# Niema-Lab/AmpliPy

Hardware: AMD Instinct MI355X
Metric: aligned reads/s through trim+pileup+call, 30 kb ref @ 10k x depth (higher is better)
Workload: dtype u8/int32

## Files before the change

amplipy_amd/csrc/amp_bf.hpp:

```cpp
#pragma once

#include "amp_read.hpp"

namespace amp {

struct Bf {
    int32_t a, m1, k, m2, c, kind;
    uint32_t op;
    uint32_t punt;
    AMP_HD int32_t kI() const { return kind == 1 ? k : 0; }
    AMP_HD int32_t kD() const { return kind == 2 ? k : 0; }
    AMP_HD int32_t query_len() const { return a + m1 + kI() + m2 + c; }
    AMP_HD int32_t ref_len() const { const int32_t r = m1 + m2 + kD(); return r ? r : 1; }
};
AMP_HD int32_t bf_sel(bool c, int32_t x, int32_t y) { return c ? x : y; }
AMP_HD int32_t bf_min(int32_t x, int32_t y) { return x < y ? x : y; }
AMP_HD int32_t bf_max(int32_t x, int32_t y) { return x > y ? x : y; }
AMP_HD Bf bf_pick(bool c, const Bf &x, const Bf &y) {
    return Bf{c ? x.a : y.a, c ? x.m1 : y.m1, c ? x.k : y.k, c ? x.m2 : y.m2, c ? x.c : y.c, c ? x.kind : y.kind, c ? x.op : y.op, c ? x.punt : y.punt};
}
AMP_HD Bf bf_mirror(const Bf &s) { return Bf{s.c, s.kind ? s.m2 : s.m1, s.k, s.kind ? s.m1 : s.m2, s.a, s.kind, s.op, s.punt}; }

AMP_HD Bf bf_from_words5(int n, uint32_t w0, uint32_t w1, uint32_t w2, uint32_t w3, uint32_t w4, int32_t lseq, int32_t max_ins, int32_t max_del, bool &ok) {
    const bool lead = (w0 & 15u) == OP_S;
// ... 31 lines not shown
    r = in2 ? s.a + s.m1 + s.kI() + u : r;
    r = inD ? s.a + s.m1 : r;
    r = in1 ? s.a + t : r;
    return r;
}

AMP_HD int32_t bf_ref_offset(const Bf &s, int32_t qp) {
    const bool in0 = (s.a > 0) & (qp <= s.a);
    const int32_t x = qp - s.a;
    const bool in1 = !in0 & (s.m1 > 0) & (x <= s.m1);
    const int32_t x2 = x - s.m1;
    const bool inI = !in0 & !in1 & (s.kind == 1) & (x2 <= s.k);
    const int32_t x3 = x2 - s.kI();
    const bool in2 = !in0 & !in1 & !inI & (s.kind != 0) & (s.m2 > 0) & (x3 <= s.m2);
    int32_t r = s.m1 + s.kD() + (s.kind ? s.m2 : 0);
    r = in2 ? s.m1 + s.kD() + x3 : r;
    r = inI ? s.m1 : r;
    r = in1 ? x : r;
    r = in0 ? 0 : r;
    return r;
}

template <bool QUALITY>
AMP_HD Bf bf_clip_left(const Bf &s, int32_t d, int32_t &adv) {
    const bool r1 = (s.m1 > 0) & (d < s.m1);
    const int32_t d1 = d - s.m1, A = s.a + s.m1;
    const bool stopI = !r1 & (s.kind == 1) & (d1 < s.k) & (QUALITY | (d1 > 0));
    const bool stopD = !r1 & (s.kind == 2) & (d1 == 0) & QUALITY;
    const bool stop = stopI | stopD;
    const int32_t d2 = s.kind == 1 ? bf_max(d1 - s.k, 0) : d1;
    const int32_t m = s.kind ? s.m2 : 0;
    const int32_t t = bf_min(d2, m);
    const int32_t m_left = m - t;
    const int32_t A4 = A + s.kI() + t;
    Bf o;
    o.op = s.op;
    o.punt = s.punt | ((!r1 & (s.kind != 0) & (s.m2 == 0)) ? 1u : 0u);
    o.a = r1 ? s.a + d : (stop ? A + (stopI ? d1 : 0) : A4 + (m_left == 0 ? s.c : 0));
    o.m1 = r1 ? s.m1 - d : (stop ? 0 : m_left);
    o.k = r1 ? s.k : (stop ? s.k - (stopI ? d1 : 0) : 0);
    o.m2 = (r1 | stop) ? s.m2 : 0;
    o.kind = (r1 | stop) ? s.kind : 0;
    o.c = (r1 | stop) ? s.c : (m_left == 0 ? 0 : s.c);
    adv = r1 ? d : (stop ? s.m1 : s.m1 + s.kD() + t);
    return o;
}

AMP_HD Bf bf_primer_clip(const Bf &s, int32_t del, int32_t &adv) {
    const int32_t d = s.a > 0 ? bf_max(del - s.a, 0) : del;
    int32_t adv_c;
    const Bf c = bf_clip_left<false>(s, bf_max(d, 0), adv_c);
    const bool neg = del < 0, zero = del == 0;
    Bf o;
    o.op = s.op;
    o.punt = (neg | zero) ? s.punt : c.punt;
    o.a = neg ? s.query_len() : (zero ? s.a : c.a);
    o.m1 = neg ? 0 : (zero ? s.m1 : c.m1);
    o.k = neg ? 0 : (zero ? s.k : c.k);
    o.m2 = neg ? 0 : (zero ? s.m2 : c.m2);
    o.c = neg ? 0 : (zero ? s.c : c.c);
    o.kind = neg ? 0 : (zero ? s.kind : c.kind);
    adv = neg ? s.kD() : (zero ? 0 : adv_c);
    return o;
}
AMP_HD Bf bf_canon(const Bf &s) {
    const bool all = (s.kind == 0) & (s.m1 == 0);
    Bf o = s;
    o.a = all ? s.a + s.c : s.a;
    o.c = all ? 0 : s.c;
    return o;
}

AMP_HD Bf bf_trim_primers(const Bf &s0, int32_t &pos, uint32_t &flags, uint32_t flag, bool isize_flag, int32_t lseq,
                          int32_t left_max_end, int32_t right_min_start) {
    const bool is_paired = flag & 1u, is_reverse = (flag & 0x10u) != 0;
    const bool do1 = !(is_paired & isize_flag & is_reverse) & (left_max_end >= 0);
    int32_t adv1;
    const Bf c1 = bf_primer_clip(s0, bf_pos_on_query(s0, left_max_end + 1 - pos), adv1);
    Bf s = bf_pick(do1, c1, s0);
    pos += do1 ? adv1 : 0;
    flags |= do1 ? AMP_TRIM_PRIMER_START : 0u;
    const bool do2 = !(is_paired & isize_flag & !is_reverse) & (right_min_start >= 0) & !s.punt;
    const int32_t del2 = lseq - bf_pos_on_query(s, right_min_start - pos);
    int32_t adv2;
    const Bf c2 = bf_canon(bf_mirror(bf_primer_clip(bf_mirror(s), del2, adv2)));
    flags |= do2 ? AMP_TRIM_PRIMER_END : 0u;
    return bf_pick(do2, c2, s);
}

AMP_HD void bf_quality_window(const Bf &s, int32_t lseq, int32_t &lo, int32_t &qlen) {
    const bool single = (s.m1 == 0) & (s.kind == 0);
    const int32_t qe = single ? lseq : lseq - s.c;
    lo = bf_min(s.a, lseq);
    qlen = bf_max(qe, lo) - lo;
}

AMP_HD Bf bf_trim_quality(const Bf &s, int32_t pos, uint32_t &flags, bool is_reverse, int32_t i, int32_t qlen) {
    int32_t adv;
    const int32_t del_r = i;
    const bool do_r = is_reverse & (bf_ref_offset(s, del_r + s.a - 1) > 0);
    const Bf cr = bf_clip_left<true>(s, del_r, adv);
    const Bf cr0 = bf_pick(del_r == 0, s, cr);
    const int32_t del_f = qlen - i;
    const bool do_f = !is_reverse & (del_f != 0);
    const Bf cf = bf_canon(bf_mirror(bf_clip_left<true>(bf_mirror(s), del_f, adv)));
    flags |= (do_r | do_f) ? AMP_TRIM_QUALITY : 0u;
    (void)pos;
    return bf_pick(do_r, cr0, bf_pick(do_f, cf, s));
}

}
```

amplipy_amd/csrc/amp_fast.hpp:

```cpp
#pragma once

#include "amp_tile.hpp"
#include "amp_bf.hpp"

namespace amp {

#ifndef AMP_F_LDSPAD
#define AMP_F_LDSPAD 0
#endif
#ifndef AMP_F4_LEAN
#define AMP_F4_LEAN 1
#endif
#ifndef AMP_F4_BF
#define AMP_F4_BF 1
#endif
__device__ __forceinline__ Bf bf_of(const Cig2 &s) { return Bf{s.a, s.m1, s.k, s.m2, s.c, s.kind, s.op, s.punt ? 1u : 0u}; }
__device__ __forceinline__ Cig2 cig2_of(const Bf &b) { return Cig2{b.op, b.a, b.m1, b.k, b.m2, b.c, b.kind, b.punt != 0u}; }
constexpr int F_NP = 10;
constexpr int F_MAXLEN = 152;
constexpr int F_PW = 256;
#ifndef AMP_F_REPS
#define AMP_F_REPS 8
#endif
constexpr int F_REP = AMP_F_REPS;
// ... 170 lines not shown
    const uint32_t se0 = __builtin_amdgcn_perm(0x00000010u, 0x00080018u, (sq.x >> 4) & 0x07070707u);
    const uint32_t so0 = __builtin_amdgcn_perm(0x00000010u, 0x00080018u, sq.x & 0x07070707u);
    const uint32_t se1 = __builtin_amdgcn_perm(0x00000010u, 0x00080018u, (sq.y >> 4) & 0x07070707u);
    const uint32_t so1 = __builtin_amdgcn_perm(0x00000010u, 0x00080018u, sq.y & 0x07070707u);
    const uint32_t f0 = nibble_to_bytes(m, 0), f1 = nibble_to_bytes(m, 1), f2 = nibble_to_bytes(m, 2), f3 = nibble_to_bytes(m, 3);
    const uint32_t wb = wrep + (inwin ? (uint32_t)d0 * 4u : 0u);
#define F_SH(d, sh, js, v, jv) "v_lshlrev_b32_sdwa " d ", " sh ", " v " dst_sel:DWORD dst_unused:UNUSED_PAD src0_sel:BYTE_" #js " src1_sel:BYTE_" #jv "\n\t"
#define F_AD(t, off) "ds_add_u32 %2, " t " offset:" #off "\n\t"
    {
        uint32_t t0, t1;
        asm volatile(F_SH("%0", "%3", 0, "%7", 0) F_SH("%1", "%4", 0, "%7", 1) F_AD("%0", 0) F_SH("%0", "%3", 1, "%7", 2) F_AD("%1", 4) F_SH("%1", "%4", 1, "%7", 3)
                     F_AD("%0", 8) F_SH("%0", "%3", 2, "%8", 0) F_AD("%1", 12) F_SH("%1", "%4", 2, "%8", 1) F_AD("%0", 16) F_SH("%0", "%3", 3, "%8", 2)
                     F_AD("%1", 20) F_SH("%1", "%4", 3, "%8", 3) F_AD("%0", 24) F_SH("%0", "%5", 0, "%9", 0) F_AD("%1", 28) F_SH("%1", "%6", 0, "%9", 1)
                     F_AD("%0", 32) F_SH("%0", "%5", 1, "%9", 2) F_AD("%1", 36) F_SH("%1", "%6", 1, "%9", 3) F_AD("%0", 40) F_SH("%0", "%5", 2, "%10", 0)
                     F_AD("%1", 44) F_SH("%1", "%6", 2, "%10", 1) F_AD("%0", 48) F_SH("%0", "%5", 3, "%10", 2) F_AD("%1", 52) F_SH("%1", "%6", 3, "%10", 3)
                     F_AD("%0", 56) "ds_add_u32 %2, %1 offset:60"
                     : "=&v"(t0), "=&v"(t1) : "v"(wb), "v"(se0), "v"(so0), "v"(se1), "v"(so1), "v"(f0), "v"(f1), "v"(f2), "v"(f3) : "memory");
    }
#undef F_SH
#undef F_AD
    return redo ? 1u : 0u;
}
__device__ __forceinline__ uint32_t count_piece5q(const uint2 &sq, uint32_t m16, int32_t d0, int32_t lim16, uint32_t wrep, uint32_t ooff) {
    const bool inwin = (d0 >= 0) & (d0 <= lim16);
    const bool redo = (m16 != 0u) & (!inwin | (nibbles_bad(sq.x, sq.y) != 0u));
    const uint32_t m = redo ? 0u : m16;
    const uint32_t se0 = __builtin_amdgcn_perm(0x00000010u, 0x00080018u, (sq.x >> 4) & 0x07070707u);
    const uint32_t so0 = __builtin_amdgcn_perm(0x00000010u, 0x00080018u, sq.x & 0x07070707u);
    const uint32_t se1 = __builtin_amdgcn_perm(0x00000010u, 0x00080018u, (sq.y >> 4) & 0x07070707u);
    const uint32_t so1 = __builtin_amdgcn_perm(0x00000010u, 0x00080018u, sq.y & 0x07070707u);
    const uint32_t f0 = nibble_to_bytes(m, 0), f1 = nibble_to_bytes(m, 1), f2 = nibble_to_bytes(m, 2), f3 = nibble_to_bytes(m, 3);
    const uint32_t wb = wrep + (inwin ? (uint32_t)d0 * 4u + (((uint32_t)d0 & 1u) ? ooff : 0u) : 0u);
#define F_SH(d, sh, js, v, jv) "v_lshlrev_b32_sdwa " d ", " sh ", " v " dst_sel:DWORD dst_unused:UNUSED_PAD src0_sel:BYTE_" #js " src1_sel:BYTE_" #jv "\n\t"
#define F_AQ(t, off) "ds_add_u64 %0, " t " offset:" #off "\n\t"
    asm volatile(F_SH("v252", "%1", 0, "%5", 0) F_SH("v253", "%2", 0, "%5", 1) F_AQ("v[252:253]", 0)
                 F_SH("v254", "%1", 1, "%5", 2) F_SH("v255", "%2", 1, "%5", 3) F_AQ("v[254:255]", 8)
                 F_SH("v252", "%1", 2, "%6", 0) F_SH("v253", "%2", 2, "%6", 1) F_AQ("v[252:253]", 16)
                 F_SH("v254", "%1", 3, "%6", 2) F_SH("v255", "%2", 3, "%6", 3) F_AQ("v[254:255]", 24)
                 F_SH("v252", "%3", 0, "%7", 0) F_SH("v253", "%4", 0, "%7", 1) F_AQ("v[252:253]", 32)
                 F_SH("v254", "%3", 1, "%7", 2) F_SH("v255", "%4", 1, "%7", 3) F_AQ("v[254:255]", 40)
                 F_SH("v252", "%3", 2, "%8", 0) F_SH("v253", "%4", 2, "%8", 1) F_AQ("v[252:253]", 48)
                 F_SH("v254", "%3", 3, "%8", 2) F_SH("v255", "%4", 3, "%8", 3) "ds_add_u64 %0, v[254:255] offset:56"
                 : : "v"(wb), "v"(se0), "v"(so0), "v"(se1), "v"(so1), "v"(f0), "v"(f1), "v"(f2), "v"(f3) : "memory", "v252", "v253", "v254", "v255");
#undef F_SH
#undef F_AQ
    return redo ? 1u : 0u;
}
__device__ __forceinline__ uint32_t range_bits16(int32_t klo, int32_t khi) {
    klo = klo < 0 ? 0 : (klo > 16 ? 16 : klo); khi = khi > 16 ? 16 : (khi < 0 ? 0 : khi);
    return ((1u << khi) - 1u) & ~((1u << klo) - 1u);
}

#if defined(AMP_DEV) && (!defined(AMP_ABL) || defined(AMP_ABL_STAMPS))
#define F_DBG_PARAM , uint32_t *f_dbg
#define F_GLOB ++f_glob
#define F_EPIW(k) do { __builtin_amdgcn_s_waitcnt(0x4F74); f_epw[0] = wall_clock64(); __builtin_amdgcn_s_waitcnt(0x0F7A); f_epw[1] = wall_clock64(); __builtin_amdgcn_s_waitcnt(0); f_ep[k] = wall_clock64(); } while (0)
#define F_EPI(k) do { __builtin_amdgcn_s_waitcnt(0); f_ep[k] = wall_clock64(); } while (0)
#define F_DBG_ARG(x) , (x)
#define F_STAMP_DECL unsigned long long f_t[8] = {0, 0, 0, 0, 0, 0, 0, 0}, f_prev = __builtin_amdgcn_s_memtime(); const unsigned long long f_k0 = f_prev, f_w0 = wall_clock64(); unsigned long long f_ep[3] = {0, 0, 0}, f_epw[2] = {0, 0}; uint32_t f_glob = 0
#define F_STAMP(k) do { __builtin_amdgcn_sched_barrier(0); __builtin_amdgcn_s_waitcnt(0xC07F); unsigned long long f_n = __builtin_amdgcn_s_memtime(); f_t[k] += f_n - f_prev; f_prev = f_n; __builtin_amdgcn_sched_barrier(0); } while (0)
#define F_STAMP_VM(k) do { __builtin_amdgcn_sched_barrier(0); __builtin_amdgcn_s_waitcnt(0x0070); unsigned long long f_n = __builtin_amdgcn_s_memtime(); f_t[k] += f_n - f_prev; f_prev = f_n; __builtin_amdgcn_sched_barrier(0); } while (0)
#define F_STAMP_OUT do { f_t[0] = __builtin_amdgcn_s_memtime() - f_k0; const unsigned long long f_w1 = wall_clock64(); f_t[7] = f_w1 - f_w0; if (lane == 0) { unsigned long long *const ctr = late_ctr(); for (int k = 0; k < 8; ++k) atomicAdd(&ctr[CTR_PHASE0 + k], f_t[k]); \
    atomicMax(&ctr[CTR_STAMP0], f_t[7]); atomicMax(&ctr[CTR_STAMP0 + 1], ~f_t[7]); atomicMax(&ctr[CTR_STAMP0 + 2], ~f_w0); atomicMax(&ctr[CTR_STAMP0 + 3], f_w1); \
    if (f_dbg && wave == 0) { uint32_t *f_o = f_dbg + blockIdx.x * 8; f_o[0] = (uint32_t)f_t[7]; f_o[1] = (uint32_t)f_w0; for (int k = 1; k < 7; ++k) f_o[1 + k] = (uint32_t)(f_t[k] >> 4); } \
    if (f_dbg) { uint32_t *f_o = f_dbg + F_DBG_WAVE0 + (blockIdx.x * F_WAVES + wave) * F_DBG_WAVEWORDS; f_o[0] = (uint32_t)((f_t[1] + f_t[2] + f_t[3] + f_t[4] + f_t[5] + f_t[6]) >> 4); f_o[1] = (uint32_t)(f_epw[0] - f_w0); f_o[2] = (uint32_t)(f_epw[1] - f_epw[0]); f_o[3] = (uint32_t)(f_ep[0] - f_epw[1]); f_o[4] = (uint32_t)(f_ep[1] - f_ep[0]); f_o[5] = (uint32_t)(f_ep[2] - f_ep[1]); } } } while (0)
#else
#define F_DBG_PARAM
#define F_DBG_ARG(x)
#define F_GLOB
// ... 4 lines not shown
#define F_STAMP_VM(k)
#define F_STAMP_OUT
#endif

#define F_ARGS \
    const int32_t *a_pos, int32_t a_min_quality, const uint16_t *a_flag, int32_t a_window, const int32_t *a_tlen, int32_t a_do_trim, \
    const uint32_t *a_lseq, int32_t a_do_count, const uint32_t *a_cig_off32, int32_t a_ref_len, const uint32_t *a_cig, int32_t a_max_primer_len, \
    const uint32_t *a_seq_off8, int32_t reads_per_block, const uint8_t *a_seq, int32_t a_epoch, const uint8_t *a_qual, int32_t pad1, \
    const int32_t *a_min_start, int32_t pad2, const int32_t *a_max_end, int32_t pad3, \
    int32_t *a_new_pos, int32_t pad4, uint32_t *a_new_ncig, int32_t pad5, uint32_t *a_new_cig, int32_t pad6, int32_t *a_o_ref_len, int32_t pad7, \
    uint8_t *a_trim_flags, int32_t pad8, uint8_t *a_status, int32_t pad9, \
    uint32_t *counts, int32_t pad10, amp_ins_event *a_ev, int32_t pad11, unsigned long long *a_ctr, int32_t pad12, uint32_t *a_ins_at, int32_t pad13, \
    uint32_t *glist, int32_t pad14, uint32_t *gcnt, int32_t pad15, \
    int64_t a_n_reads, int32_t pad17, uint64_t read_base, int32_t pad18, long long a_ev_cap
#define F_ARGS_PASS(P, rd, out, eb, rpb) \
    (rd).pos, (P).min_quality, (rd).flag, (P).window, (rd).tlen, (P).do_trim, (rd).lseq, (P).do_count, (rd).cig_off32, (P).ref_len, (rd).cig, \
    (P).max_primer_len, (rd).seq_off8, (rpb), (rd).seq, (int32_t)(P).epoch, (rd).qual, 0, (P).min_start, 0, (P).max_end, 0, (out).new_pos, 0, (out).new_ncig, 0, \
    (out).new_cig, 0, (out).ref_len, 0, (out).trim_flags, 0, (out).status, 0, counts, 0, (eb).ev, 0, (eb).ctr, 0, (eb).ins_at, 0, glist, 0, gcnt, 0, \
    (rd).n_reads, 0, read_base, 0, (eb).cap

enum : uint32_t { KA_MIN_START = 144, KA_MAX_END = 160, KA_NEW_POS = 176, KA_NEW_NCIG = 192, KA_NEW_CIG = 208, KA_O_REF_LEN = 224, KA_TRIM_FLAGS = 240,
                  KA_STATUS = 256, KA_COUNTS = 272, KA_EV = 288, KA_CTR = 304, KA_INS_AT = 320, KA_GLIST = 336, KA_GCNT = 352, KA_N_READS = 368,
                  KA_READ_BASE = 384, KA_EV_CAP = 400 };
template <typename T>
__device__ __forceinline__ T karg_late(uint32_t off) {
    static_assert(sizeof(T) == 8, "the late-loaded arguments are pointers and 64-bit values");
    asm volatile("" : "+s"(off));
    const unsigned long long v = *(const __attribute__((address_space(4))) unsigned long long *)
        ((const __attribute__((address_space(4))) uint8_t *)__builtin_amdgcn_kernarg_segment_ptr() + off);
    return __builtin_bit_cast(T, v);
}
template <typename T>
__device__ __forceinline__ T *karg_late_ptr(uint32_t off) {
    return (T *)karg_late<__attribute__((address_space(1))) T *>(off);
}

#if AMP_F_ADD64
#define F_COUNT5(sq, m, d0, lim, wr) count_piece5q(sq, m, d0, lim, wr, (uint32_t)(F_REPW * 4))
#else
#define F_COUNT5(sq, m, d0, lim, wr) count_piece5(sq, m, d0, lim, wr)
#endif
template <int W>
__global__ void __launch_bounds__(F_WAVES * 64, 2)
k_fast(F_ARGS F_DBG_PARAM) {
    const KParams P{a_min_quality, a_window, a_do_trim, a_do_count, a_ref_len, a_max_primer_len, nullptr, nullptr, (uint32_t)a_epoch};
    const amp_dev_reads rd{a_n_reads, a_pos, a_flag, a_tlen, a_lseq, a_cig_off32, a_cig, a_seq_off8, a_seq, a_qual, 0, 0};
    auto late_ctr = [] { return karg_late_ptr<unsigned long long>(KA_CTR); };
    auto late_eb = [] { return EventBuf{karg_late_ptr<amp_ins_event>(KA_EV), karg_late_ptr<unsigned long long>(KA_CTR), karg_late_ptr<uint32_t>(KA_INS_AT), karg_late<long long>(KA_EV_CAP)}; };
    __shared__ uint4 s_stage[F_WAVES][(F_PAD + F_STAGE + 16) / 16];
    __shared__ __attribute__((aligned(8))) uint32_t s_pwin[F_WAVES][F_REP * F_REPW];
    __shared__ uint32_t s_bwin[F_BPL * F_BW];
    __shared__ uint32_t s_ticket, s_gcur;
#if AMP_F_LDSPAD > 0
    __shared__ uint32_t s_pad[AMP_F_LDSPAD / 4];
    if (P.ref_len == -12345) s_pad[threadIdx.x] = 1;
#endif
    const int tid = threadIdx.x, wave = tid >> 6, lane = tid & 63;
    F_STAMP_DECL;
    const int64_t n = rd.n_reads;
    const int64_t rb = (int64_t)blockIdx.x * reads_per_block;
    const int64_t re = rb + reads_per_block < n ? rb + reads_per_block : n;
    lds_u32 *const bwin = (lds_u32 *)s_bwin;
    lds_u32 *const pwin = (lds_u32 *)s_pwin[wave];
    for (int i = tid; i < F_BPL * F_BW; i += F_WAVES * 64) bwin[i] = 0;
    for (int i = lane; i < F_REP * F_REPW; i += 64) pwin[i] = 0;
    if (lane < F_PAD / 4) ((lds_u32 *)s_stage[wave])[lane] = 0x11111111u;
    if (tid == 0) { s_ticket = 0; s_gcur = 0; }
    if (tid == 0 && blockIdx.x == 0) { unsigned long long *const ctr = late_ctr(); ctr[CTR_LONG_N] = 0ull; ctr[CTR_LONG_TICKET] = 0ull; ctr[CTR_GEN_LEFT] = 0ull; }
    int32_t bw_base = rb < n ? rd.pos[rb] : 0;
    bw_base = (bw_base < 16 ? 0 : bw_base - 16) & ~15;
    __syncthreads();

    const int32_t mq = P.min_quality;
    const uint32_t mqc = (uint32_t)(mq > 256 ? 256 : mq);
    const uint32_t thr = mqc * (uint32_t)W;
    const uint32_t mqb = (uint32_t)mq * 0x01010101u;
    const uint32_t G = (uint32_t)P.ref_len;
    const uint32_t n_tb = re > rb ? (uint32_t)((re - rb + 63) / 64) : 0u;
    auto take_ticket = [&]() {
        uint32_t t = 0;
        if (lane == 0) t = __hip_atomic_fetch_add((lds_u32 *)&s_ticket, 1u, __ATOMIC_RELAXED, __HIP_MEMORY_SCOPE_WORKGROUP);
        return (uint32_t)__builtin_amdgcn_readfirstlane((int)t);
    };
    const int64_t wend = re;
    unsigned long long n_err = 0;
#ifndef AMP_F_REPSHIFT
#define AMP_F_REPSHIFT 2
#endif
    const uint32_t rep = (F_REP & (F_REP - 1)) ? ((uint32_t)lane >> AMP_F_REPSHIFT) % (uint32_t)F_REP : ((uint32_t)lane >> AMP_F_REPSHIFT) & (uint32_t)(F_REP - 1);
    const uint32_t phi_lane = ((uint32_t)lane >> 1) & 1u ? 8u : 0u;
#if AMP_F_ADD64
    lds_u8 *const wrep = (lds_u8 *)pwin + (rep & (uint32_t)(F_REP / 2 - 1)) * (uint32_t)(2 * F_REPW * 4);
    static_assert((F_REP & 1) == 0 && (F_REPW & 1) == 1, "two arrays per replica, the second one an odd number of words behind the first");
#else
    lds_u8 *const wrep = (lds_u8 *)pwin + rep * (uint32_t)(F_REPW * 4);
#endif
    lds_u8 *const stage = (lds_u8 *)s_stage[wave] + F_PAD;
    int32_t pw_base = 0;
    int pw_tiles = F_FLUSH;
    const unsigned ev_shard = blockIdx.x & (EV_SHARDS - 1);
    unsigned long long ev_base = 0;
    uint32_t ev_left = 0;

    auto fold = [&]() {
        asm volatile("s_waitcnt lgkmcnt(0)" ::: "memory");
        wave_sync();
#pragma unroll 1
        for (int idx = lane; idx < F_PW; idx += 64) {
// ... 80 lines not shown
        g.Tq = g.solo ? 0u : (uint32_t)__builtin_amdgcn_readlane((int)(g.row + 8u * nch), g.ntake - 1);
        g.fastq = g.taken && shortq;
        return g;
    };
    auto shape_of = [&](const HdrP &h, const Cg &c, bool fastq) {
        Shape r;
#if AMP_F4_BF
        bool ok;
        r.s = cig2_of(bf_from_words5((int)h.nops(), c.w[0], c.w[1], c.w[2], c.w[3], c.w[4], fastq ? (int32_t)h.lseq() : 0, F_MAXINS, F_MAXDEL, ok));
        r.ok = ok;
#else
        r.s = Cig2{0u, 0, 0, 0, 0, 0, 0, false};
        const int nops = (int)h.nops();
        r.ok = fastq && nops >= 1 && nops <= 5 && cig2_from_words5(nops, c.w, (int32_t)h.lseq(), r.s);
        if (r.ok && ((r.s.kind == 1 && r.s.k > F_MAXINS) || (r.s.kind == 2 && r.s.k > F_MAXDEL))) r.ok = false;
        if (!r.ok) r.s = Cig2{0u, 0, 0, 0, 0, 0, 0, false};
#endif
        r.refspan = r.ok ? r.s.m1 + r.s.m2 + (r.s.kind == 2 ? r.s.k : 0) : 1;
        return r;
    };
    auto load_tabs = [&](const HdrP &h, const Shape &sh, bool trim) {
        Tabs t{-1, -1};
        const bool in_ref = (uint32_t)h.pos < G && (uint32_t)(h.pos + sh.refspan - 1) < G;
        if (trim && in_ref) { t.L = karg_late_ptr<const int32_t>(KA_MAX_END)[h.pos]; t.R = karg_late_ptr<const int32_t>(KA_MIN_START)[h.pos + sh.refspan - 1]; }
        return t;
    };
    auto issue_bytes = [&](const Geo &g, uint32_t m0) {
        Bytes x;
        const uint8_t *qrun = rd.qual + (int64_t)m0 * 8;
        const uint8_t *srun = rd.seq + (int64_t)m0 * 4;
        const uint32_t lastq = g.Tq ? (g.Tq - 1u) & ~15u : 0u, lasts = g.Tq ? ((g.Tq >> 1) - 1u) & ~15u : 0u;
#pragma unroll
        for (int sl = 0; sl < F_STAGE / 1024; ++sl) {
            uint32_t off = (uint32_t)(sl * 1024 + lane * 16);
            off = off < lastq ? off : lastq;
            __builtin_amdgcn_global_load_lds((const __attribute__((address_space(1))) void *)(qrun + off),
                                             (__attribute__((address_space(3))) void *)(stage + sl * 1024), 16, 0, 0);
        }
#pragma unroll
        for (int sl = 0; sl < F_STAGE / 2048; ++sl) {
            uint32_t off = (uint32_t)(sl * 1024 + lane * 16);
            off = off < lasts ? off : lasts;
            const uint32_t *sp = (const uint32_t *)(srun + off);
            x.raws[sl] = make_uint4(sp[0], sp[1], sp[2], sp[3]);
        }
        return x;
    };
    enum : uint32_t { P_STORED = 1u << 24, P_LIST = 1u << 25, P_STATUS_ONLY = 1u << 26 };
    struct Pend { uint32_t i, slot_lo; int32_t pos, reflen; uint32_t meta, cw0, cw1, cw2, cw3, cw4; };
    Pend pend{0u, 0u, 0, 0, 0u, 0u, 0u, 0u, 0u, 0u};
    auto store_pending = [&](const Pend &r) {
#if defined(AMP_DEV) && defined(AMP_ABL)
        if (AMP_ABL & 8) return;
#endif
        const uint32_t ncig = r.meta & 0xFFu;
        if (r.meta & P_STORED) {
            const DevOut out{karg_late_ptr<int32_t>(KA_NEW_POS), karg_late_ptr<uint32_t>(KA_NEW_NCIG), karg_late_ptr<uint32_t>(KA_NEW_CIG),
                             karg_late_ptr<int32_t>(KA_O_REF_LEN), karg_late_ptr<uint8_t>(KA_TRIM_FLAGS), karg_late_ptr<uint8_t>(KA_STATUS)};
            uint32_t *home = out.new_cig + ((size_t)r.slot_lo + 3 * (size_t)r.i);
            if (ncig > 0u) home[0] = r.cw0;
            if (ncig > 1u) home[1] = r.cw1;
            if (ncig > 2u) home[2] = r.cw2;
            if (ncig > 3u) home[3] = r.cw3;
            if (ncig > 4u) home[4] = r.cw4;
            if (out.new_pos) out.new_pos[r.i] = r.pos;
            if (out.new_ncig) out.new_ncig[r.i] = ncig;
            if (out.ref_len) out.ref_len[r.i] = r.reflen;
            if (out.trim_flags) out.trim_flags[r.i] = (uint8_t)(r.meta >> 16);
            if (out.status) out.status[r.i] = (uint8_t)(r.meta >> 8);
        }
        const bool has = (r.meta & P_LIST) != 0;
        const unsigned long long m = __ballot(has);
        if (m) {
            uint32_t base = 0;
            if (lane == 0) base = __hip_atomic_fetch_add((lds_u32 *)&s_gcur, (uint32_t)__popcll(m), __ATOMIC_RELAXED, __HIP_MEMORY_SCOPE_WORKGROUP);
            base = (uint32_t)__builtin_amdgcn_readfirstlane((int)base);
            if (has) karg_late_ptr<uint32_t>(KA_GLIST)[(size_t)rb + base + __popcll(m & ((1ull << lane) - 1ull))] = r.i | ((r.meta & P_STATUS_ONLY) ? GL_STATUS_ONLY : 0u);
        }
    };

    uint32_t pw_lim = 0;
// ... 146 lines not shown
        if (do_trim_t && !(AMP_ABL & 4)) {
#else
        if (do_trim_t) {
#endif
#pragma unroll
            for (int k = 0; k < F_NP; ++k) {
                uint32_t p = (uint32_t)k + rot;
                p = p >= np ? p - np : p;
                p = (uint32_t)k < np ? p : np;
                const int32_t j0 = (int32_t)(p * 16u);
                uint2 nx = make_uint2(q16[0].x, q16[0].y);
                if (k + 1 < F_NP && (uint32_t)(k + 1) < np) nx = make_uint2(q16[k + 1].x, q16[k + 1].y);
                uint32_t fail = piece_fail_bits<W>(q16[k], nx, thr);
                int32_t blo = lo - j0, bhi = hi - W - j0;
                blo = blo < 0 ? 0 : (blo > 16 ? 16 : blo); bhi = bhi > 15 ? 15 : (bhi < -1 ? -1 : bhi);
                fail &= (0xFFFFu >> (15 - bhi)) & (0xFFFFu << blo);
                const int32_t f1 = j0 + (__builtin_ffs((int)fail) - 1), e1 = j0 + (31 - __builtin_clz(fail)) + W;
                ffmin = fail && f1 < ffmin ? f1 : ffmin;
                lemax = fail && e1 > lemax ? e1 : lemax;
            }
        }

        F_STAMP(3);
        bool general = i < re && !shaped;
        bool stored = false;
        uint32_t ncig = 0, cw[5] = {0u, 0u, 0u, 0u, 0u};
        int32_t reflen = 0;
        if (shaped) {
            if (fb == 0xFFu || s.punt) {
                general = true;
            } else {
                if (scan) {
                    int32_t iq;
                    if (!rev && ffmin != 0x7FFFFFFF) iq = ffmin - lo;
                    else if (rev && lemax >= 0) iq = lemax - lo;
                    else {
                        iq = rev ? 0 : qlen;
                        int32_t acc = 0;
                        const uint64_t t_lo = (uint64_t)tw0.x | ((uint64_t)tw0.y << 32), t_hi = (uint64_t)tw1.x | ((uint64_t)tw1.y << 32);
                        const int32_t kmax = qlen < W - 1 ? qlen : W - 1;
                        const int32_t qlo = lo - (int32_t)phi, qhi = hi - (int32_t)phi;
                        for (int32_t k = 1; k <= kmax; ++k) {
                            const uint32_t o = (uint32_t)((rev ? qlo + k - 1 : qhi - k) - tab);
                            acc += (int32_t)(((o < 8u ? t_lo : t_hi) >> ((o & 7u) * 8u)) & 0xFFu);
                            if ((int64_t)acc < (int64_t)mq * k) iq = rev ? k : qlen - k;
                        }
                    }
#if AMP_F4_BF
                    { uint32_t f2 = ts.flags; s = cig2_of(bf_trim_quality(bf_of(s), ts.pos, f2, rev, iq, qlen)); ts.flags = f2; }
#else
                    cig2_trim_quality(ts, rev, iq, qlen, s);
#endif
                }
                if (s.punt) {
                    general = true;
                } else {
                    if (!ts.err) {
                        const uint32_t part[5] = {((uint32_t)s.a << 4) | OP_S, ((uint32_t)s.m1 << 4) | s.op,
                                                  ((uint32_t)s.k << 4) | (s.kind == 1 ? OP_I : OP_D), ((uint32_t)s.m2 << 4) | s.op,
                                                  ((uint32_t)s.c << 4) | OP_S};
                        const bool has[5] = {s.a > 0, s.m1 > 0, s.kind != 0, s.kind != 0 && s.m2 > 0, s.c > 0};
#pragma unroll
                        for (int t = 0; t < 5; ++t) {
                            if (has[t]) {
#pragma unroll
                                for (int j = (t == 3 ? 1 : 0); j <= t; ++j) cw[j] = ncig == (uint32_t)j ? part[t] : cw[j];
                                ++ncig;
                            }
                        }
                        reflen = s.ref_len();
                    }
                    stored = true;
                    if (ts.err) ++n_err;
                }
            }
        }
        const bool counted = stored && !ts.err && do_count_t;
        F_STAMP(4);
        const bool two = counted && s.kind != 0;
        const int32_t qa1 = counted ? s.a + (int32_t)phi : 0, qb1 = counted ? qa1 + s.m1 : 0;
        const int32_t qa2 = two ? qb1 + (s.kind == 1 ? s.k : 0) : qb1, qb2 = two ? qa2 + s.m2 : qa2;
        const int32_t pos2 = ts.pos + s.m1 + (s.kind == 2 ? s.k : 0);
        bool bad_extra = false;
        if (two && s.kind == 2) {
            for (int32_t j = 0; j < s.k; ++j) {
                const int32_t r = ts.pos + s.m1 + j;
                const uint32_t d = (uint32_t)(r - bw_base);
                if ((uint32_t)r >= G) bad_extra = true;
                else if (d < (uint32_t)F_BW) lds_add_nt(bwin + 4 * F_BW + d, 1u);
                else atomicAdd(&karg_late_ptr<uint32_t>(KA_COUNTS)[(size_t)r * AMP_NSYM + 5], 1u);
            }
        }
        {
            uint32_t good = 0;
            if (two && s.kind == 1) {
                const uint32_t o0 = ok_bits4(iq0.x, mqb) >> 7, o1 = ok_bits4(iq0.y, mqb) >> 7, o2 = ok_bits4(iq1.x, mqb) >> 7, o3 = ok_bits4(iq1.y, mqb) >> 7;
                auto nib = [](uint32_t o) { return ((o * 0x00204081u) >> 21) & 0xFu; };
                const uint32_t m16 = nib(o0) | (nib(o1) << 4) | (nib(o2) << 8) | (nib(o3) << 12);
                good = (m16 >> (uint32_t)(s.a + s.m1 - g_ins)) & ((1u << s.k) - 1u);
// ... 28 lines not shown
                        if (firstrun) {
                            if ((long long)slot < eb.cap) eb.ev[(size_t)ev_shard * (size_t)eb.cap + slot] = inside ? amp_ins_event{ins_pos, rid, elo, ehi} : amp_ins_event{-1, 0u, 0, 0};
                            if (inside) {
                                const uint32_t d = (uint32_t)(ins_pos - bw_base);
                                if (d < (uint32_t)F_BW) lds_add_nt(bwin + 5 * F_BW + d, 1u);
                                else atomicAdd(&eb.ins_at[ins_pos], 1u);
                            }
                        } else if (inside) {
                            eb.record(ins_pos, rid, elo, ehi);
                        }
                        firstrun = false;
                    }
                }
                ev_base += total; ev_left -= total;
            }
        }
        uint32_t redo = 0;
#if AMP_F4_LEAN
        uint32_t okm[F_NP];
#pragma unroll
        for (int k = 0; k < F_NP; ++k) okm[k] = ok_bits16(q16[k], mqb);
        const uint32_t okB = ok_bits16(make_uint4(bq0.x, bq0.y, bq1.x, bq1.y), mqb);
#endif
        int32_t xbe = 0, jb = 0;
        bool has_b = false;
        if (two) {
            const int32_t jstar = (qb1 - 1) & ~15;
            has_b = jstar + 16 > qa2 && qb2 > qa2;
            xbe = qb2 < jstar + 16 ? qb2 : jstar + 16;
            jb = g_b + (int32_t)phi;
        }
        const int32_t end_pos = two ? pos2 + s.m2 : ts.pos + s.m1;
        bool todo = counted;
#if defined(AMP_DEV) && defined(AMP_ABL)
        if (AMP_ABL & 2) todo = false;
#endif
        for (bool first_pass = true;; first_pass = false) {
            const unsigned long long tm = __ballot(todo);
            if (!tm) break;
            const int lead = __builtin_ctzll(tm);
            if (!first_pass) {
                fold();
                const int32_t lead_pos = __builtin_amdgcn_readlane(pos, lead);
                pw_base = (lead_pos < 16 ? 0 : lead_pos - 16) & ~15; pw_tiles = 1;
                pw_lim = (int64_t)G - pw_base >= (int64_t)F_PW ? (uint32_t)F_PW : (uint32_t)(G > (uint32_t)pw_base ? G - (uint32_t)pw_base : 0u);
            }
            const bool fits = ts.pos - pw_base >= 16 && end_pos - pw_base + 16 <= (int32_t)pw_lim;
            const bool now = todo && (fits || lane == lead);
            const int32_t a1 = now ? qa1 : 0, b1 = now ? qb1 : 0, a2 = now ? qa2 : 0, b2 = now ? qb2 : 0;
            const int32_t dbase1 = ts.pos - pw_base - qa1, dbase2 = pos2 - pw_base - qa2;
#if AMP_F4_LEAN
            const int32_t lim16 = (int32_t)pw_lim - 16;
            if (__ballot(has_b && now)) {
                const uint32_t mB = (has_b & now) ? okB & range_bits16(qa2 - jb, xbe - jb) : 0u;
// ... 64 lines not shown
    store_pending(pend);
    pad_events();
    F_EPI(1);
    if (pw_tiles && n_tb) fold();
    F_EPI(2);
    asm volatile("s_waitcnt lgkmcnt(0)" ::: "memory");
    __syncthreads();
#if defined(AMP_DEV) && defined(AMP_ABL)
    if (AMP_ABL & 16) return;
#endif
    uint32_t *const counts_l = karg_late_ptr<uint32_t>(KA_COUNTS), *const ins_at_l = karg_late_ptr<uint32_t>(KA_INS_AT);
    for (int i = tid; i < F_BPL * F_BW; i += F_WAVES * 64) {
        const uint32_t v = bwin[i];
        if (v) {
            const int pl = i / F_BW, d = i - pl * F_BW;
            const uint32_t p = (uint32_t)(bw_base + d);
            if (p < G) {
                if (pl < F_NPL) atomicAdd(&counts_l[(size_t)p * AMP_NSYM + pl], v);
                else if (pl == 4) atomicAdd(&counts_l[(size_t)p * AMP_NSYM + 5], v);
                else atomicAdd(&ins_at_l[p], v);
            }
        }
    }
    if (n_err) atomicAdd(&late_ctr()[CTR_ERROR_READS], n_err);
    F_STAMP_OUT;
    if (tid == 0) { karg_late_ptr<uint32_t>(KA_GCNT)[blockIdx.x] = s_gcur; if (s_gcur) late_ctr()[CTR_EPOCH] = (unsigned long long)P.epoch; }
}

__global__ void __launch_bounds__(256)
k_gcompact(const uint32_t *__restrict__ glist, const uint32_t *__restrict__ gcnt, int reads_per_block, int64_t n_reads,
           uint32_t *__restrict__ dense, GenGeo *geo, uint32_t gen_grid, unsigned long long *ctr,
           const uint32_t *__restrict__ cig_off32, uint32_t *__restrict__ llist, uint32_t *__restrict__ lpos, int long_max_ops) {
    __shared__ uint32_t s_part[4], s_lw[4], s_lbase;
    const int tid = threadIdx.x;
    uint32_t acc = 0;
    for (int b = tid; b < (int)blockIdx.x; b += 256) acc += gcnt[b];
    for (int o = 32; o > 0; o >>= 1) acc += __shfl_down(acc, o);
    if ((tid & 63) == 0) s_part[tid >> 6] = acc;
    __syncthreads();
    const uint32_t off = s_part[0] + s_part[1] + s_part[2] + s_part[3];
    const uint32_t cnt = gcnt[blockIdx.x];
    const int64_t sbeg = (int64_t)blockIdx.x * reads_per_block;
    const uint32_t *src = glist + (sbeg < n_reads ? sbeg : 0);
    for (uint32_t k = tid; k < cnt; k += 256) dense[off + k] = src[k];
    if (long_max_ops) {
        const auto kind = [&](uint32_t k) -> uint32_t {
            if (k >= cnt) return 0u;
// ... 68 lines not shown
```

Before: 10.31 billion.

## Branchless trim/CIGAR packing, shared clip path, and paired kernarg pointer loads

Rewrites the breakpoint-form clip and trim helpers so the primer and quality trims run one clip instead of two and select between results. The mirror is made conditional, so forward and reverse share one code path. Turns the per-read CIGAR word emission and the quality-scan branching into straight-line predicated code, and fetches pairs of late kernel-argument pointers with a single 32-byte scalar load. The aim is less divergence, fewer instructions and fewer scalar loads per read, at the cost of subtle semantic equivalence risk in the clip logic and always running the quality trim math.

```diff
diff --git a/amplipy_amd/csrc/amp_bf.hpp b/amplipy_amd/csrc/amp_bf.hpp
--- a/amplipy_amd/csrc/amp_bf.hpp
+++ b/amplipy_amd/csrc/amp_bf.hpp
@@ -77,45 +77,34 @@
 }
 
 template <bool QUALITY>
-AMP_HD Bf bf_clip_left(const Bf &s, int32_t d, int32_t &adv) {
-    const bool r1 = (s.m1 > 0) & (d < s.m1);
-    const int32_t d1 = d - s.m1, A = s.a + s.m1;
-    const bool stopI = !r1 & (s.kind == 1) & (d1 < s.k) & (QUALITY | (d1 > 0));
-    const bool stopD = !r1 & (s.kind == 2) & (d1 == 0) & QUALITY;
-    const bool stop = stopI | stopD;
-    const int32_t d2 = s.kind == 1 ? bf_max(d1 - s.k, 0) : d1;
-    const int32_t m = s.kind ? s.m2 : 0;
-    const int32_t t = bf_min(d2, m);
-    const int32_t m_left = m - t;
-    const int32_t A4 = A + s.kI() + t;
+AMP_HD Bf bf_clip_left(const Bf &s, int32_t d, bool skip, int32_t &adv) {
+    const int32_t kI = s.kI(), kD = s.kD();
+    const int32_t e = bf_min(d, s.m1), d1 = d - e;
+    const int32_t kq = QUALITY ? (s.kind == 2 ? 1 : kI) : kI;
+    const bool keep = QUALITY ? ((d < s.m1 + kq) | skip) : (((d < s.m1 + kq) & (d != s.m1)) | skip);
+    const int32_t t = bf_min(bf_max(d1 - kI, 0), s.m2);
+    const int32_t m_left = s.m2 - t;
+    const bool gone = m_left == 0;
     Bf o;
     o.op = s.op;
-    o.punt = s.punt | ((!r1 & (s.kind != 0) & (s.m2 == 0)) ? 1u : 0u);
-    o.a = r1 ? s.a + d : (stop ? A + (stopI ? d1 : 0) : A4 + (m_left == 0 ? s.c : 0));
-    o.m1 = r1 ? s.m1 - d : (stop ? 0 : m_left);
-    o.k = r1 ? s.k : (stop ? s.k - (stopI ? d1 : 0) : 0);
-    o.m2 = (r1 | stop) ? s.m2 : 0;
-    o.kind = (r1 | stop) ? s.kind : 0;
-    o.c = (r1 | stop) ? s.c : (m_left == 0 ? 0 : s.c);
-    adv = r1 ? d : (stop ? s.m1 : s.m1 + s.kD() + t);
+    o.punt = s.punt | (((d >= s.m1) & !skip & (s.kind != 0) & (s.m2 == 0)) ? 1u : 0u);
+    o.a = keep ? s.a + d : s.a + s.m1 + kI + t + (gone ? s.c : 0);
+    o.m1 = keep ? s.m1 - e : m_left;
+    o.k = keep ? s.k - d1 : 0;
+    o.m2 = keep ? s.m2 : 0;
+    o.kind = keep ? s.kind : 0;
+    o.c = (keep | !gone) ? s.c : 0;
+    adv = keep ? e : s.m1 + kD + t;
     return o;
 }
 
 AMP_HD Bf bf_primer_clip(const Bf &s, int32_t del, int32_t &adv) {
-    const int32_t d = s.a > 0 ? bf_max(del - s.a, 0) : del;
+    const bool neg = del < 0, zero = del == 0;
+    const int32_t d = neg ? 0x3FFFFFFF : bf_max(del - s.a, 0);
     int32_t adv_c;
-    const Bf c = bf_clip_left<false>(s, bf_max(d, 0), adv_c);
-    const bool neg = del < 0, zero = del == 0;
-    Bf o;
-    o.op = s.op;
-    o.punt = (neg | zero) ? s.punt : c.punt;
-    o.a = neg ? s.query_len() : (zero ? s.a : c.a);
-    o.m1 = neg ? 0 : (zero ? s.m1 : c.m1);
-    o.k = neg ? 0 : (zero ? s.k : c.k);
-    o.m2 = neg ? 0 : (zero ? s.m2 : c.m2);
-    o.c = neg ? 0 : (zero ? s.c : c.c);
-    o.kind = neg ? 0 : (zero ? s.kind : c.kind);
-    adv = neg ? s.kD() : (zero ? 0 : adv_c);
+    Bf o = bf_clip_left<false>(s, d, zero, adv_c);
+    o.punt = neg ? s.punt : o.punt;
+    adv = neg ? s.kD() : adv_c;
     return o;
 }
 AMP_HD Bf bf_canon(const Bf &s) {
@@ -125,43 +114,41 @@
     o.c = all ? 0 : s.c;
     return o;
 }
+AMP_HD Bf bf_mirror_if(bool f, const Bf &s) {
+    const bool sw = f & (s.kind != 0);
+    return Bf{f ? s.c : s.a, sw ? s.m2 : s.m1, s.k, sw ? s.m1 : s.m2, f ? s.a : s.c, s.kind, s.op, s.punt};
+}
 
 AMP_HD Bf bf_trim_primers(const Bf &s0, int32_t &pos, uint32_t &flags, uint32_t flag, bool isize_flag, int32_t lseq,
                           int32_t left_max_end, int32_t right_min_start) {
     const bool is_paired = flag & 1u, is_reverse = (flag & 0x10u) != 0;
-    const bool do1 = !(is_paired & isize_flag & is_reverse) & (left_max_end >= 0);
+    const bool far = is_paired & isize_flag;
+    const bool do1 = !(far & is_reverse) & (left_max_end >= 0);
     int32_t adv1;
-    const Bf c1 = bf_primer_clip(s0, bf_pos_on_query(s0, left_max_end + 1 - pos), adv1);
-    Bf s = bf_pick(do1, c1, s0);
-    pos += do1 ? adv1 : 0;
+    const Bf s = bf_primer_clip(s0, do1 ? bf_pos_on_query(s0, left_max_end + 1 - pos) : 0, adv1);
+    pos += adv1;
     flags |= do1 ? AMP_TRIM_PRIMER_START : 0u;
-    const bool do2 = !(is_paired & isize_flag & !is_reverse) & (right_min_start >= 0) & !s.punt;
-    const int32_t del2 = lseq - bf_pos_on_query(s, right_min_start - pos);
+    const bool do2 = !(far & !is_reverse) & (right_min_start >= 0) & !s.punt;
+    const int32_t del2 = do2 ? lseq - bf_pos_on_query(s, right_min_start - pos) : 0;
     int32_t adv2;
-    const Bf c2 = bf_canon(bf_mirror(bf_primer_clip(bf_mirror(s), del2, adv2)));
     flags |= do2 ? AMP_TRIM_PRIMER_END : 0u;
-    return bf_pick(do2, c2, s);
+    return bf_canon(bf_mirror(bf_primer_clip(bf_mirror(s), del2, adv2)));
 }
 
 AMP_HD void bf_quality_window(const Bf &s, int32_t lseq, int32_t &lo, int32_t &qlen) {
-    const bool single = (s.m1 == 0) & (s.kind == 0);
-    const int32_t qe = single ? lseq : lseq - s.c;
     lo = bf_min(s.a, lseq);
-    qlen = bf_max(qe, lo) - lo;
+    qlen = bf_max(lseq - s.c, lo) - lo;
 }
 
 AMP_HD Bf bf_trim_quality(const Bf &s, int32_t pos, uint32_t &flags, bool is_reverse, int32_t i, int32_t qlen) {
     int32_t adv;
-    const int32_t del_r = i;
-    const bool do_r = is_reverse & (bf_ref_offset(s, del_r + s.a - 1) > 0);
-    const Bf cr = bf_clip_left<true>(s, del_r, adv);
-    const Bf cr0 = bf_pick(del_r == 0, s, cr);
-    const int32_t del_f = qlen - i;
-    const bool do_f = !is_reverse & (del_f != 0);
-    const Bf cf = bf_canon(bf_mirror(bf_clip_left<true>(bf_mirror(s), del_f, adv)));
-    flags |= (do_r | do_f) ? AMP_TRIM_QUALITY : 0u;
+    const bool fwd = !is_reverse;
+    const int32_t del = fwd ? qlen - i : i;
+    const bool doit = fwd ? del != 0 : bf_ref_offset(s, del + s.a - 1) > 0;
+    flags |= doit ? AMP_TRIM_QUALITY : 0u;
+    const int32_t d = doit ? del : 0;
     (void)pos;
-    return bf_pick(do_r, cr0, bf_pick(do_f, cf, s));
+    return bf_canon(bf_mirror_if(fwd, bf_clip_left<true>(bf_mirror_if(fwd, s), d, d == 0, adv)));
 }
 
 }
diff --git a/amplipy_amd/csrc/amp_fast.hpp b/amplipy_amd/csrc/amp_fast.hpp
--- a/amplipy_amd/csrc/amp_fast.hpp
+++ b/amplipy_amd/csrc/amp_fast.hpp
@@ -216,9 +216,9 @@
     return redo ? 1u : 0u;
 }
 __device__ __forceinline__ uint32_t count_piece5q(const uint2 &sq, uint32_t m16, int32_t d0, int32_t lim16, uint32_t wrep, uint32_t ooff) {
-    const bool inwin = (d0 >= 0) & (d0 <= lim16);
-    const bool redo = (m16 != 0u) & (!inwin | (nibbles_bad(sq.x, sq.y) != 0u));
-    const uint32_t m = redo ? 0u : m16;
+    const bool inwin = (uint32_t)d0 < (lim16 < 0 ? 0u : (uint32_t)lim16 + 1u);
+    const uint32_t defect = inwin ? nibbles_bad(sq.x, sq.y) : 1u;
+    const uint32_t m = defect ? 0u : m16;
     const uint32_t se0 = __builtin_amdgcn_perm(0x00000010u, 0x00080018u, (sq.x >> 4) & 0x07070707u);
     const uint32_t so0 = __builtin_amdgcn_perm(0x00000010u, 0x00080018u, sq.x & 0x07070707u);
     const uint32_t se1 = __builtin_amdgcn_perm(0x00000010u, 0x00080018u, (sq.y >> 4) & 0x07070707u);
@@ -238,7 +238,8 @@
                  : : "v"(wb), "v"(se0), "v"(so0), "v"(se1), "v"(so1), "v"(f0), "v"(f1), "v"(f2), "v"(f3) : "memory", "v252", "v253", "v254", "v255");
 #undef F_SH
 #undef F_AQ
-    return redo ? 1u : 0u;
+    const uint32_t left = m16 ^ m;
+    return left < 1u ? left : 1u;
 }
 __device__ __forceinline__ uint32_t range_bits16(int32_t klo, int32_t khi) {
     klo = klo < 0 ? 0 : (klo > 16 ? 16 : klo); khi = khi > 16 ? 16 : (khi < 0 ? 0 : khi);
@@ -289,6 +290,8 @@
 enum : uint32_t { KA_MIN_START = 144, KA_MAX_END = 160, KA_NEW_POS = 176, KA_NEW_NCIG = 192, KA_NEW_CIG = 208, KA_O_REF_LEN = 224, KA_TRIM_FLAGS = 240,
                   KA_STATUS = 256, KA_COUNTS = 272, KA_EV = 288, KA_CTR = 304, KA_INS_AT = 320, KA_GLIST = 336, KA_GCNT = 352, KA_N_READS = 368,
                   KA_READ_BASE = 384, KA_EV_CAP = 400 };
+static_assert(KA_MAX_END == KA_MIN_START + 16 && KA_NEW_NCIG == KA_NEW_POS + 16 && KA_O_REF_LEN == KA_NEW_CIG + 16 && KA_STATUS == KA_TRIM_FLAGS + 16 &&
+              KA_CTR == KA_EV + 16, "karg_late2 reads two neighbours");
 template <typename T>
 __device__ __forceinline__ T karg_late(uint32_t off) {
     static_assert(sizeof(T) == 8, "the late-loaded arguments are pointers and 64-bit values");
@@ -297,9 +300,21 @@
         ((const __attribute__((address_space(4))) uint8_t *)__builtin_amdgcn_kernarg_segment_ptr() + off);
     return __builtin_bit_cast(T, v);
 }
+struct KargPair { unsigned long long a, b; };
+__device__ __forceinline__ KargPair karg_late2(uint32_t off) {
+    typedef unsigned long long amp_u64x4 __attribute__((ext_vector_type(4), aligned(16)));
+    asm volatile("" : "+s"(off));
+    const amp_u64x4 v = *(const __attribute__((address_space(4))) amp_u64x4 *)
+        ((const __attribute__((address_space(4))) uint8_t *)__builtin_amdgcn_kernarg_segment_ptr() + off);
+    return KargPair{v.x, v.z};
+}
 template <typename T>
 __device__ __forceinline__ T *karg_late_ptr(uint32_t off) {
     return (T *)karg_late<__attribute__((address_space(1))) T *>(off);
+}
+template <typename T>
+__device__ __forceinline__ T *karg_ptr_of(unsigned long long v) {
+    return (T *)__builtin_bit_cast(__attribute__((address_space(1))) T *, v);
 }
 
 #if AMP_F_ADD64
@@ -313,7 +328,10 @@
     const KParams P{a_min_quality, a_window, a_do_trim, a_do_count, a_ref_len, a_max_primer_len, nullptr, nullptr, (uint32_t)a_epoch};
     const amp_dev_reads rd{a_n_reads, a_pos, a_flag, a_tlen, a_lseq, a_cig_off32, a_cig, a_seq_off8, a_seq, a_qual, 0, 0};
     auto late_ctr = [] { return karg_late_ptr<unsigned long long>(KA_CTR); };
-    auto late_eb = [] { return EventBuf{karg_late_ptr<amp_ins_event>(KA_EV), karg_late_ptr<unsigned long long>(KA_CTR), karg_late_ptr<uint32_t>(KA_INS_AT), karg_late<long long>(KA_EV_CAP)}; };
+    auto late_eb = [] {
+        const KargPair ec = karg_late2(KA_EV);
+        return EventBuf{karg_ptr_of<amp_ins_event>(ec.a), karg_ptr_of<unsigned long long>(ec.b), karg_late_ptr<uint32_t>(KA_INS_AT), karg_late<long long>(KA_EV_CAP)};
+    };
     __shared__ uint4 s_stage[F_WAVES][(F_PAD + F_STAGE + 16) / 16];
     __shared__ __attribute__((aligned(8))) uint32_t s_pwin[F_WAVES][F_REP * F_REPW];
     __shared__ uint32_t s_bwin[F_BPL * F_BW];
@@ -350,7 +368,7 @@
         return (uint32_t)__builtin_amdgcn_readfirstlane((int)t);
     };
     const int64_t wend = re;
-    unsigned long long n_err = 0;
+    uint32_t n_err = 0;
 #ifndef AMP_F_REPSHIFT
 #define AMP_F_REPSHIFT 2
 #endif
@@ -477,7 +495,10 @@
     auto load_tabs = [&](const HdrP &h, const Shape &sh, bool trim) {
         Tabs t{-1, -1};
         const bool in_ref = (uint32_t)h.pos < G && (uint32_t)(h.pos + sh.refspan - 1) < G;
-        if (trim && in_ref) { t.L = karg_late_ptr<const int32_t>(KA_MAX_END)[h.pos]; t.R = karg_late_ptr<const int32_t>(KA_MIN_START)[h.pos + sh.refspan - 1]; }
+        if (trim && in_ref) {
+            const KargPair tabs = karg_late2(KA_MIN_START);
+            t.L = karg_ptr_of<const int32_t>(tabs.b)[h.pos]; t.R = karg_ptr_of<const int32_t>(tabs.a)[h.pos + sh.refspan - 1];
+        }
         return t;
     };
     auto issue_bytes = [&](const Geo &g, uint32_t m0) {
@@ -510,8 +531,9 @@
 #endif
         const uint32_t ncig = r.meta & 0xFFu;
         if (r.meta & P_STORED) {
-            const DevOut out{karg_late_ptr<int32_t>(KA_NEW_POS), karg_late_ptr<uint32_t>(KA_NEW_NCIG), karg_late_ptr<uint32_t>(KA_NEW_CIG),
-                             karg_late_ptr<int32_t>(KA_O_REF_LEN), karg_late_ptr<uint8_t>(KA_TRIM_FLAGS), karg_late_ptr<uint8_t>(KA_STATUS)};
+            const KargPair o01 = karg_late2(KA_NEW_POS), o23 = karg_late2(KA_NEW_CIG), o45 = karg_late2(KA_TRIM_FLAGS);
+            const DevOut out{karg_ptr_of<int32_t>(o01.a), karg_ptr_of<uint32_t>(o01.b), karg_ptr_of<uint32_t>(o23.a),
+                             karg_ptr_of<int32_t>(o23.b), karg_ptr_of<uint8_t>(o45.a), karg_ptr_of<uint8_t>(o45.b)};
             uint32_t *home = out.new_cig + ((size_t)r.slot_lo + 3 * (size_t)r.i);
             if (ncig > 0u) home[0] = r.cw0;
             if (ncig > 1u) home[1] = r.cw1;
@@ -704,59 +726,39 @@
         }
 
         F_STAMP(3);
-        bool general = i < re && !shaped;
-        bool stored = false;
-        uint32_t ncig = 0, cw[5] = {0u, 0u, 0u, 0u, 0u};
-        int32_t reflen = 0;
-        if (shaped) {
-            if (fb == 0xFFu || s.punt) {
-                general = true;
-            } else {
-                if (scan) {
-                    int32_t iq;
-                    if (!rev && ffmin != 0x7FFFFFFF) iq = ffmin - lo;
-                    else if (rev && lemax >= 0) iq = lemax - lo;
-                    else {
-                        iq = rev ? 0 : qlen;
-                        int32_t acc = 0;
-                        const uint64_t t_lo = (uint64_t)tw0.x | ((uint64_t)tw0.y << 32), t_hi = (uint64_t)tw1.x | ((uint64_t)tw1.y << 32);
-                        const int32_t kmax = qlen < W - 1 ? qlen : W - 1;
-                        const int32_t qlo = lo - (int32_t)phi, qhi = hi - (int32_t)phi;
-                        for (int32_t k = 1; k <= kmax; ++k) {
-                            const uint32_t o = (uint32_t)((rev ? qlo + k - 1 : qhi - k) - tab);
-                            acc += (int32_t)(((o < 8u ? t_lo : t_hi) >> ((o & 7u) * 8u)) & 0xFFu);
-                            if ((int64_t)acc < (int64_t)mq * k) iq = rev ? k : qlen - k;
-                        }
-                    }
+        const bool star = fb == 0xFFu;
+        int32_t iq = rev ? (lemax >= 0 ? lemax - lo : 0) : (ffmin != 0x7FFFFFFF ? ffmin - lo : qlen);
+        const bool tail = scan & (rev ? lemax < 0 : ffmin == 0x7FFFFFFF);
+        if (tail) {
+            int32_t acc = 0;
+            const uint64_t t_lo = (uint64_t)tw0.x | ((uint64_t)tw0.y << 32), t_hi = (uint64_t)tw1.x | ((uint64_t)tw1.y << 32);
+            const int32_t kmax = qlen < W - 1 ? qlen : W - 1;
+            const int32_t qlo = lo - (int32_t)phi, qhi = hi - (int32_t)phi;
+            for (int32_t k = 1; k <= kmax; ++k) {
+                const uint32_t o = (uint32_t)((rev ? qlo + k - 1 : qhi - k) - tab);
+                acc += (int32_t)(((o < 8u ? t_lo : t_hi) >> ((o & 7u) * 8u)) & 0xFFu);
+                if ((int64_t)acc < (int64_t)mq * k) iq = rev ? k : qlen - k;
+            }
+        }
 #if AMP_F4_BF
-                    { uint32_t f2 = ts.flags; s = cig2_of(bf_trim_quality(bf_of(s), ts.pos, f2, rev, iq, qlen)); ts.flags = f2; }
+        { uint32_t f2 = ts.flags; s = cig2_of(bf_trim_quality(bf_of(s), ts.pos, f2, rev, iq, qlen)); ts.flags = f2; }
 #else
-                    cig2_trim_quality(ts, rev, iq, qlen, s);
-#endif
-                }
-                if (s.punt) {
-                    general = true;
-                } else {
-                    if (!ts.err) {
-                        const uint32_t part[5] = {((uint32_t)s.a << 4) | OP_S, ((uint32_t)s.m1 << 4) | s.op,
-                                                  ((uint32_t)s.k << 4) | (s.kind == 1 ? OP_I : OP_D), ((uint32_t)s.m2 << 4) | s.op,
-                                                  ((uint32_t)s.c << 4) | OP_S};
-                        const bool has[5] = {s.a > 0, s.m1 > 0, s.kind != 0, s.kind != 0 && s.m2 > 0, s.c > 0};
-#pragma unroll
-                        for (int t = 0; t < 5; ++t) {
-                            if (has[t]) {
-#pragma unroll
-                                for (int j = (t == 3 ? 1 : 0); j <= t; ++j) cw[j] = ncig == (uint32_t)j ? part[t] : cw[j];
-                                ++ncig;
-                            }
-                        }
-                        reflen = s.ref_len();
-                    }
-                    stored = true;
-                    if (ts.err) ++n_err;
-                }
-            }
-        }
+        if (scan) cig2_trim_quality(ts, rev, iq, qlen, s);
+#endif
+        const bool stored = shaped & !star & !s.punt;
+        const bool general = i < re && !stored;
+        const bool emit = stored & (ts.err == 0);
+        const bool has0 = emit & (s.a > 0), has1 = emit & (s.m1 > 0), has2 = emit & (s.kind != 0), has3 = has2 & (s.m2 > 0), has4 = emit & (s.c > 0);
+        uint32_t cw[5] = {((uint32_t)s.a << 4) | OP_S, ((uint32_t)s.m1 << 4) | s.op, ((uint32_t)s.k << 4) | (s.kind == 1 ? OP_I : OP_D),
+                          ((uint32_t)s.m2 << 4) | s.op, ((uint32_t)s.c << 4) | OP_S};
+        cw[4] = has4 ? cw[4] : 0u;
+        cw[3] = has3 ? cw[3] : cw[4]; cw[4] = has3 ? cw[4] : 0u;
+        cw[2] = has2 ? cw[2] : cw[3]; cw[3] = has2 ? cw[3] : cw[4]; cw[4] = has2 ? cw[4] : 0u;
+        cw[1] = has1 ? cw[1] : cw[2]; cw[2] = has1 ? cw[2] : cw[3]; cw[3] = has1 ? cw[3] : cw[4]; cw[4] = has1 ? cw[4] : 0u;
+        cw[0] = has0 ? cw[0] : cw[1]; cw[1] = has0 ? cw[1] : cw[2]; cw[2] = has0 ? cw[2] : cw[3]; cw[3] = has0 ? cw[3] : cw[4]; cw[4] = has0 ? cw[4] : 0u;
+        const uint32_t ncig = (has0 ? 1u : 0u) + (has1 ? 1u : 0u) + (has2 ? 1u : 0u) + (has3 ? 1u : 0u) + (has4 ? 1u : 0u);
+        const int32_t reflen = emit ? s.ref_len() : 0;
+        n_err += (stored & (ts.err != 0)) ? 1u : 0u;
         const bool counted = stored && !ts.err && do_count_t;
         F_STAMP(4);
         const bool two = counted && s.kind != 0;
@@ -831,14 +833,9 @@
         for (int k = 0; k < F_NP; ++k) okm[k] = ok_bits16(q16[k], mqb);
         const uint32_t okB = ok_bits16(make_uint4(bq0.x, bq0.y, bq1.x, bq1.y), mqb);
 #endif
-        int32_t xbe = 0, jb = 0;
-        bool has_b = false;
-        if (two) {
-            const int32_t jstar = (qb1 - 1) & ~15;
-            has_b = jstar + 16 > qa2 && qb2 > qa2;
-            xbe = qb2 < jstar + 16 ? qb2 : jstar + 16;
-            jb = g_b + (int32_t)phi;
-        }
+        const int32_t jstar = (qb1 - 1) & ~15;
+        const bool has_b = two & (jstar + 16 > qa2) & (qb2 > qa2);
+        const int32_t xbe = qb2 < jstar + 16 ? qb2 : jstar + 16, jb = g_b + (int32_t)phi;
         const int32_t end_pos = two ? pos2 + s.m2 : ts.pos + s.m1;
         bool todo = counted;
 #if defined(AMP_DEV) && defined(AMP_ABL)
@@ -949,7 +946,7 @@
             }
         }
     }
-    if (n_err) atomicAdd(&late_ctr()[CTR_ERROR_READS], n_err);
+    if (n_err) atomicAdd(&late_ctr()[CTR_ERROR_READS], (unsigned long long)n_err);
     F_STAMP_OUT;
     if (tid == 0) { karg_late_ptr<uint32_t>(KA_GCNT)[blockIdx.x] = s_gcur; if (s_gcur) late_ctr()[CTR_EPOCH] = (unsigned long long)P.epoch; }
 }
```

New measurement: 10.69 billion (median of 6 runs). 1.04x the previous value.
